# Lexmata/llama-gguf

Measured on AMD Instinct MI355X. Metric: decode tokens/sec Llama-3-8B Q4_K_M, 1 GPU; % of HBM roofline, higher is better.
Workload: dtype f32 (x as 4xint8 limbs on the matrix cores, exact int32 accumulation)

## Files before the change

### llama-gguf_amd/csrc/attention.hip

```cpp
#include <cstdlib>

#include "attn_split.h"
#include "tq_fwht.h"
#include "xq.h"
#include "prefill.h"
#include "timeline.h"

LGH_TL_DEFINE(attn)

namespace lgh {

template <int D, int G, int NW, bool PF = false, bool DIRECT = false, bool MULTI = false>
__global__ void __launch_bounds__(NW * 64) attn_partial_kernel(const float* __restrict__ q, const float* __restrict__ kc,
                                                           const float* __restrict__ vc, uint32_t max_seq, float scale,
                                                           const int* pos_ptr, int kv_len_fixed, uint32_t n_splits,
                                                           float* __restrict__ part_ml, float* __restrict__ part_acc,
                                                           const int* __restrict__ slot = nullptr, uint64_t slot_stride = 0) {
  constexpr int LPR = D / 4;
  constexpr int RPW = 64 / LPR;
  __shared__ float s_ml[NW * G * 2];
  __shared__ __attribute__((aligned(16))) float s_acc[NW * G * D];
  LGH_TL_BEGIN(attn, lgh::TL_ATTN, n_splits);

  const uint32_t kvh = blockIdx.x / n_splits, sp = blockIdx.x % n_splits;
  const uint32_t lane = threadIdx.x & 63, wave = threadIdx.x >> 6;
  const uint32_t sub = lane / LPR, li = lane % LPR;
  uint32_t kv_len = (uint32_t)kv_len_fixed;
  if (PF) {
    kv_len += blockIdx.y;
    q += (size_t)blockIdx.y * gridDim.x * G * D;
  } else if (MULTI) {
    const uint32_t sq = blockIdx.y;
    uint32_t pw, sl;
    sload_u32x2(pos_ptr + sq, slot + sq, pw, sl);
    kv_len = pw + 1;
    q += (size_t)sq * (gridDim.x / n_splits) * G * D;
    kc += (size_t)sl * slot_stride;
    vc += (size_t)sl * slot_stride;
    part_ml += (size_t)sq * gridDim.x * G * 2;
    part_acc += (size_t)sq * gridDim.x * G * D;
  } else if (pos_ptr) {
    kv_len = sload_u32(pos_ptr) + 1;
  }

  f32x4 qv[G];
#pragma unroll
  for (int g = 0; g < G; g++) qv[g] = *reinterpret_cast<const f32x4*>(q + ((size_t)kvh * G + g) * D + li * 4);

  float m[G], l[G];
  f32x4 acc[G];
#pragma unroll
  for (int g = 0; g < G; g++) { m[g] = kNegBig; l[g] = 0.0f; acc[g] = (f32x4)(0.0f); }

  const float* kbase = kc + (size_t)kvh * max_seq * D + li * 4;
  const float* vbase = vc + (size_t)kvh * max_seq * D + li * 4;
  const uint32_t stride = n_splits * NW * RPW;
  auto row_of = [&](uint32_t base) { const uint32_t p = base + sub; return p < kv_len ? p : kv_len - 1; };
  auto step = [&](uint32_t base, f32x4 k4, f32x4 v4) { attn_step4<G, LPR>(qv, k4, v4, scale, base + sub < kv_len, m, l, acc); };
  constexpr int kAhead = 4;
  for (uint32_t base = (sp * NW + wave) * RPW; base < kv_len; base += kAhead * stride) {
    f32x4 kk[kAhead], vv[kAhead];
#pragma unroll
    for (int j = 0; j < kAhead; j++) {
      const uint32_t r = row_of(base + j * stride);
      kk[j] = __builtin_nontemporal_load(reinterpret_cast<const f32x4*>(kbase + (size_t)r * D));
      vv[j] = __builtin_nontemporal_load(reinterpret_cast<const f32x4*>(vbase + (size_t)r * D));
    }
#pragma unroll
    for (int j = 0; j < kAhead; j++)
      if (base + j * stride < kv_len) step(base + j * stride, kk[j], vv[j]);
  }

  attn_merge_rows<G, LPR>(m, l, acc);
  attn_stash<G, 4, LPR>(s_ml, s_acc, wave, sub, li, m, l, acc);
  __syncthreads();
  const size_t pbase = ((size_t)kvh * n_splits + sp) * G;
  for (uint32_t e = threadIdx.x; e < (uint32_t)(G * D); e += NW * 64) {
    const uint32_t g = e / D, dim = e % D;
    float mn, lsum, a;
    attn_merge_waves<NW, G, D>(s_ml, s_acc, g, dim, mn, lsum, a);
    if (DIRECT) {
      const float o = a * (1.0f / lsum);
      part_acc[(pbase + g) * D + dim] = o;
      if (part_ml) xq_store_chunk(reinterpret_cast<uint8_t*>(part_ml), (uint32_t)((pbase + g) * D + dim) >> 4, o);
    } else if (PF) {
      const _Float16 o = (_Float16)(a * (1.0f / lsum));
      *reinterpret_cast<_Float16*>(reinterpret_cast<uint8_t*>(part_acc) + xh_offset(blockIdx.y, (uint32_t)(pbase + g) * D + dim)) = o;
    } else {
      attn_store_partial<D>(part_ml, part_acc, pbase + g, dim, mn, lsum, a);
    }
  }
  LGH_TL_END();
}

__device__ __forceinline__ f32x4 unpack_i8x4(uint32_t w, float scale) {
  f32x4 r;
  r.x = (float)(int)(int8_t)(w & 0xFFu) * scale;
  r.y = (float)(int)(int8_t)((w >> 8) & 0xFFu) * scale;
  r.z = (float)(int)(int8_t)((w >> 16) & 0xFFu) * scale;
  r.w = (float)(int)(int8_t)(w >> 24) * scale;
  return r;
}

__device__ __forceinline__ float i8_row_scale(float amax) { return amax > 1e-10f ? amax / 127.0f : 1.0f; }
__device__ __forceinline__ uint32_t i8_quantize(float v, float scale) {
  float r = roundf(v / scale);
  r = r < -128.0f ? -128.0f : (r > 127.0f ? 127.0f : r);
  return (uint32_t)(int)r & 0xFFu;
}

template <int LPR>
__device__ __forceinline__ uint32_t quantize_row_i8(f32x4 x, float& scale) {
  float amax = fmaxf(fmaxf(fabsf(x.x), fabsf(x.y)), fmaxf(fabsf(x.z), fabsf(x.w)));
  amax = fmaxf(amax, dpp_f<0xB1>(amax));
  amax = fmaxf(amax, dpp_f<0x4E>(amax));
  amax = fmaxf(amax, dpp_f<0x141>(amax));
  amax = fmaxf(amax, dpp_f<0x140>(amax));
  if (LPR == 32) amax = fmaxf(amax, __shfl_xor(amax, 16, 64));
  scale = i8_row_scale(amax);
  return i8_quantize(x.x, scale) | i8_quantize(x.y, scale) << 8 | i8_quantize(x.z, scale) << 16 | i8_quantize(x.w, scale) << 24;
}

template <int FMT>
__device__ __forceinline__ float fp8_decode(uint32_t b) {
  const uint32_t mag = b & 0x7Fu;
// ... 231 lines not shown
  hipStream_t st;
  uint32_t n_seq; const int* slot; uint64_t slot_stride;
};

template <int D, int G, int NW>
static hipError_t attn_go(const AttnArgs& a) {
  const dim3 grid(a.n_kv * a.n_splits, a.n_seq ? a.n_seq : 1);
  if (a.n_seq)
    hipLaunchKernelGGL((attn_partial_kernel<D, G, NW, false, false, true>), grid, dim3(NW * 64), 0, a.st, a.q, a.kc, a.vc, a.max_seq, a.scale, a.pos, 0,
                       a.n_splits, a.part_ml, a.part_acc, a.slot, a.slot_stride);
  else
    hipLaunchKernelGGL((attn_partial_kernel<D, G, NW>), grid, dim3(NW * 64), 0, a.st, a.q, a.kc, a.vc, a.max_seq, a.scale, a.pos, a.kv_len_fixed,
                       a.n_splits, a.part_ml, a.part_acc);
  return hipGetLastError();
}

static hipError_t attn_split_dispatch(uint32_t head_dim, uint32_t g, const AttnArgs& a) {
  const bool long_ctx = (a.pos ? a.max_seq : (uint32_t)a.kv_len_fixed) >= 2048;
  return attn_dispatch(head_dim, g, [&](auto d, auto gg) {
    constexpr int D = decltype(d)::value, G = decltype(gg)::value;
    return long_ctx ? attn_go<D, G, 8>(a) : attn_go<D, G, 4>(a);
  });
}

hipError_t attn_launch(const float* q, const float* kcache, const float* vcache, uint32_t n_heads, uint32_t n_kv,
                       uint32_t head_dim, uint32_t max_seq, float scale, const int* pos, int kv_len_fixed,
                       uint32_t n_splits, float* part_ml, float* part_acc, hipStream_t st) {
  if (n_kv == 0 || n_heads % n_kv) return hipErrorInvalidValue;
  return attn_split_dispatch(head_dim, n_heads / n_kv,
                             AttnArgs{q, kcache, vcache, n_kv, max_seq, scale, pos, kv_len_fixed, n_splits, part_ml, part_acc, st, 0, nullptr, 0});
}

hipError_t attn_direct_launch(const float* q, const float* kcache, const float* vcache, uint32_t n_heads, uint32_t n_kv, uint32_t head_dim,
                              uint32_t max_seq, float scale, const int* pos, float* out, uint8_t* xq_out, hipStream_t st) {
  if (n_kv == 0 || n_heads % n_kv || !pos) return hipErrorInvalidValue;
  return attn_dispatch(head_dim, n_heads / n_kv, [&](auto d, auto gg) {
    hipLaunchKernelGGL((attn_partial_kernel<decltype(d)::value, decltype(gg)::value, 16, false, true>), dim3(n_kv), dim3(1024), 0, st, q, kcache, vcache,
                       max_seq, scale, pos, 0, 1u, reinterpret_cast<float*>(xq_out), out);
    return hipGetLastError();
  });
}

struct PfTqEpi { const float* signs; float inv_scale, inv_d; };

template <int D, int NW, bool TQ>
__global__ void __launch_bounds__(NW * 64) attn_pf_mfma_kernel(const float* __restrict__ q, const float* __restrict__ kc, const float* __restrict__ vc,
                                                               uint32_t n_heads, uint32_t g_per_kv, uint32_t max_seq, float scale, uint32_t pos0,
                                                               uint32_t m_tokens, uint8_t* __restrict__ xh_out, const PfTqEpi tq) {
  constexpr int DJ = D / 4;
  constexpr int DQ = D / 16;
  constexpr int DP = D + 4;
  extern __shared__ __attribute__((aligned(16))) float pf_lds[];
  float (*s_o)[16][DP] = reinterpret_cast<float (*)[16][DP]>(pf_lds);
  float (*s_m)[16] = reinterpret_cast<float (*)[16]>(pf_lds + NW * 16 * DP);
  float (*s_l)[16] = s_m + NW;
  const uint32_t head = blockIdx.x, tt = blockIdx.y, kvh = head / g_per_kv;
  const uint32_t lane = threadIdx.x & 63, wave = threadIdx.x >> 6, n = lane & 15, c = lane >> 4;
  const uint32_t tok = tt * 16 + n, tokc = tok < m_tokens ? tok : m_tokens - 1;
  const uint32_t kv_last = pos0 + m_tokens - 1;
  const uint32_t n_tiles = (pos0 + tt * 16 + 16 + 15) / 16;
  float qf[DJ];
  {
    const float* qp = q + ((size_t)tokc * n_heads + head) * D + c * DJ;
#pragma unroll
    for (int j = 0; j < DJ; j += 4) {
      const f32x4 v = *reinterpret_cast<const f32x4*>(qp + j);
      qf[j] = v.x; qf[j + 1] = v.y; qf[j + 2] = v.z; qf[j + 3] = v.w;
    }
  }
  const float* kbase = kc + (size_t)kvh * max_seq * D;
  const float* vbase = vc + (size_t)kvh * max_seq * D;
// ... 243 lines not shown
```

### llama-gguf_amd/csrc/common.h

```cpp
#pragma once

#include <hip/hip_runtime.h>
#include <stdint.h>
#include <stddef.h>
#include <vector>

#include "../../include/llama_gguf_hip.h"

namespace lgh {

typedef uint32_t u32x4 __attribute__((ext_vector_type(4)));
typedef uint32_t u32x2 __attribute__((ext_vector_type(2)));
typedef float f32x4 __attribute__((ext_vector_type(4)));

constexpr int kWave = 64;
constexpr int kNumCU = 256;

__host__ __device__ inline uint32_t blk_elems(int t) {
  switch (t) {
    case LGH_TYPE_F32: case LGH_TYPE_F16: case LGH_TYPE_BF16: return 1;
    case LGH_TYPE_Q4_0: case LGH_TYPE_Q4_1: case LGH_TYPE_Q5_0: case LGH_TYPE_Q5_1: case LGH_TYPE_Q8_0:
    case LGH_TYPE_Q8_1: return 32;
    case LGH_TYPE_Q2_K: case LGH_TYPE_Q3_K: case LGH_TYPE_Q4_K: case LGH_TYPE_Q5_K: case LGH_TYPE_Q6_K:
    case LGH_TYPE_Q8_K: return 256;
// ... 148 lines not shown
hipError_t embed_launch(int src_type, const uint8_t* table, const int* token, float* dst, uint32_t hidden, int* state,
                        uint8_t* xq, const float* xq_nw, float* xq_ssq, hipStream_t st);

hipError_t rms_norm_launch(const float* x, const float* w, float eps, float* out, uint32_t n, hipStream_t st);
hipError_t rope_launch(float* q, float* k, uint32_t n_heads, uint32_t n_kv, uint32_t head_dim, const int* pos,
                       const float* rope_cs, int neox, hipStream_t st);
hipError_t embed_multi_launch(int src_type, const uint8_t* table, const int* tokens, float* dst, uint32_t hidden, uint32_t n_seq, uint8_t* xq,
                              const float* xq_nw, float* xq_ssq, uint32_t xq_stride, uint32_t ssq_stride, hipStream_t st);
hipError_t argmax_multi_launch(const float* logits, uint32_t n, uint32_t n_seq, float* part_val, int* part_idx, int* next, hipStream_t st);
hipError_t attn_multi_launch(const float* q, const float* kcache, const float* vcache, uint32_t n_heads, uint32_t n_kv, uint32_t head_dim,
                             uint32_t max_seq, float scale, const int* pos, const int* slot, uint64_t slot_stride, uint32_t n_seq,
                             uint32_t n_splits, float* part_ml, float* part_acc, hipStream_t st);
hipError_t attn_combine_multi_launch(const float* part_ml, const float* part_acc, uint32_t n_heads, uint32_t n_kv, uint32_t head_dim,
                                     uint32_t n_splits, uint32_t n_seq, float* out, uint8_t* xq_out, hipStream_t st);
hipError_t ewise_launch(int op, const float* a, const float* b, float s, float* out, uint64_t n, hipStream_t st);
hipError_t softmax_rows_launch(const float* x, float* out, uint32_t rows, uint32_t last_dim, hipStream_t st);
hipError_t matmul_f32_launch(const float* a, const float* b, float* c, uint32_t m, uint32_t k, uint32_t n, hipStream_t st);
hipError_t silu_mul_launch(const float* gate, const float* up, float* out, uint32_t n, hipStream_t st);
hipError_t argmax_launch(const float* logits, uint32_t n, float* part_val, int* part_idx, int* state, int* out_token,
                         hipStream_t st);
hipError_t argmax_merge_launch(const float* part_val, const int* part_idx, uint32_t nparts, int* state, int* out_token, hipStream_t st);
hipError_t advance_launch(int* state, hipStream_t st);
hipError_t copy_words_launch(void* dst, const void* src, uint32_t n_words, hipStream_t st);
hipError_t moe_group_launch(const int* sel, uint32_t n_seq, uint32_t top_k, uint32_t n_experts, int* cnt, int* idx, uint32_t idx_stride, hipStream_t st);
hipError_t moe_combine_launch(const float* tmp, const float* moe_w, uint32_t top_k, float* hidden, uint32_t H, uint32_t n_seq, const float* nw,
                              uint8_t* xq, uint32_t xq_stride, float* ssq, uint32_t ssq_stride, hipStream_t st);
hipError_t moe_router_launch(const float* x, const float* norm_w, float eps, const float* w, uint32_t hidden,
                             uint32_t n_experts, uint32_t top_k, int* sel, float* sel_w, hipStream_t st, uint32_t n_tokens = 1);

hipError_t attn_launch(const float* q, const float* kcache, const float* vcache, uint32_t n_heads, uint32_t n_kv,
                       uint32_t head_dim, uint32_t max_seq, float scale, const int* pos, int kv_len_fixed,
                       uint32_t n_splits, float* part_ml, float* part_acc, hipStream_t st);
hipError_t attn_direct_launch(const float* q, const float* kcache, const float* vcache, uint32_t n_heads, uint32_t n_kv, uint32_t head_dim,
                              uint32_t max_seq, float scale, const int* pos, float* out, uint8_t* xq_out, hipStream_t st);
bool attn_shape_has_fast_kernel(uint32_t head_dim, uint32_t group);
hipError_t kv_roundtrip_launch(int fmt, const float* x, uint32_t n, uint8_t* bytes, float* scale_out, float* back, hipStream_t st);
hipError_t attn_q8_launch(int fmt, const float* q, int8_t* k8, int8_t* v8, float* kscale, float* vscale, const float* k_new, const float* v_new,
                          uint32_t n_heads, uint32_t n_kv, uint32_t head_dim, uint32_t max_seq, float scale, const int* pos, uint32_t n_splits,
                          float* part_ml, float* part_acc, hipStream_t st);
hipError_t attn_q8_multi_launch(int fmt, const float* q, int8_t* k8, int8_t* v8, float* kscale, float* vscale, const float* k_new, const float* v_new,
                                uint32_t x_stride, uint32_t n_heads, uint32_t n_kv, uint32_t head_dim, uint32_t max_seq, float scale, const int* pos,
                                const int* slot, uint32_t n_seq, uint32_t n_splits, float* part_ml, float* part_acc, hipStream_t st);
hipError_t attn_tq_launch(int bits, const float* q, uint8_t* kq, uint8_t* vq, const float* k_new, const float* v_new, const float* signs,
                          uint32_t n_heads, uint32_t n_kv, uint32_t head_dim, uint32_t max_seq, float scale, const int* pos, uint32_t n_splits,
                          float* part_ml, float* part_acc, hipStream_t st, const float* qjl_s = nullptr, uint32_t* kx = nullptr);
hipError_t attn_tq_combine_launch(int bits, const float* part_ml, const float* part_acc, const float* signs, uint32_t n_heads, uint32_t n_kv,
                                  uint32_t head_dim, uint32_t n_splits, float* out, uint8_t* xq_out, hipStream_t st, uint32_t n_seq = 0,
                                  uint32_t xq_stride = 0);
hipError_t attn_tq_multi_launch(int bits, const float* q, uint8_t* kq, uint8_t* vq, const float* k_new, const float* v_new, const float* signs,
                                uint32_t n_heads, uint32_t n_kv, uint32_t head_dim, uint32_t max_seq, float scale, const int* pos, const int* slot,
                                uint64_t code_stride, uint64_t x_stride, uint32_t kv_stride, uint32_t n_seq, uint32_t n_splits, float* part_ml,
                                float* part_acc, hipStream_t st, const float* qjl_s = nullptr, uint32_t* kx = nullptr);
hipError_t tq_compress_launch(int bits, const float* x, uint32_t dim, const float* signs, uint8_t* out, hipStream_t st, const float* qjl_s = nullptr,
                              uint32_t* qjl_out = nullptr);
uint32_t tq_row_bytes_host(int bits, uint32_t d);
hipError_t tq_pf_rows_launch(int bits, float* kscr, float* vscr, uint8_t* kq, uint8_t* vq, float* q, const float* signs, uint32_t n_heads,
                             uint32_t n_kv, uint32_t head_dim, uint32_t max_seq, uint32_t pos0, uint32_t m_store, uint32_t m_q, uint32_t n_expand,
                             hipStream_t st);
hipError_t attn_prefill_tq_launch(const float* q, const float* kscr, const float* vscr, const float* signs, uint32_t n_heads, uint32_t n_kv,
                                  uint32_t head_dim, uint32_t max_seq, float scale, uint32_t pos0, uint32_t m_tokens, uint8_t* xh_out, hipStream_t st);
hipError_t attn_decode_any_launch(const float* q, const float* kcache, const float* vcache, float* out, uint32_t n_heads, uint32_t n_kv,
                                  uint32_t head_dim, uint32_t max_seq, float scale, const int* pos, hipStream_t st);
hipError_t attn_generic_launch(const float* q, const float* k, const float* v, float* out, uint32_t n_heads, uint32_t n_kv, uint32_t seq_len,
                               uint32_t kv_len, uint32_t kv_rows, uint32_t d, float scale, hipStream_t st);
hipError_t attn_combine_launch(const float* part_ml, const float* part_acc, uint32_t n_heads, uint32_t n_kv,
                               uint32_t head_dim, uint32_t n_splits, float* out, uint8_t* xq_out, hipStream_t st);

// ... 15 lines not shown
```

### llama-gguf_amd/csrc/engine.h

```cpp
#pragma once

#include <functional>
#include <string>
#include <vector>

#include "common.h"
#include "kv_cache.h"
#include "sample.h"

namespace lgh {

struct LayerW {
  bool owned = false;
  DevWeight wq, wk, wv, wo, gate, up, down;
  DevWeight gate_exps, up_exps, down_exps;
  float* attn_norm = nullptr;
  float* ffn_norm = nullptr;
  float* router = nullptr;
  float* bq = nullptr; float* bk = nullptr; float* bv = nullptr; float* bo = nullptr;
  KvCache kv;
  bool moe() const { return router != nullptr; }
};

enum TokenMode { MODE_PREFILL = 0, MODE_FORWARD = 1, MODE_GREEDY = 2, MODE_SAMPLE = 3, MODE_COUNT = 4 };
// ... 35 lines not shown
  SampBufs samp;
  std::vector<lgh_sampler_config_ex> samp_cfg;
  std::vector<uint8_t> samp_set;
};

}

struct lgh_ctx {
  lgh_model_desc d{};
  lgh::KvLayout kvl;
  int device = 0;
  uint32_t l0 = 0, l1 = 0;
  bool first = true, last = true;
  hipStream_t own_stream = nullptr, stream = nullptr;
  std::vector<lgh::LayerW> layers;
  uint8_t* embd_raw = nullptr;
  int embd_type = -1;
  size_t embd_bytes = 0;
  std::vector<uint8_t> embd_host;
  lgh::DevWeight output;
  float* output_norm = nullptr;
  void *fwd_hidden = nullptr, *fwd_token = nullptr;
  float *hidden = nullptr, *xnorm = nullptr, *q = nullptr, *kv_tmp = nullptr, *attn_out = nullptr, *act = nullptr,
        *act2 = nullptr, *logits = nullptr, *part_ml = nullptr, *part_acc = nullptr, *rope_cs = nullptr, *moe_w = nullptr,
        *amax_v = nullptr;
  int *moe_sel = nullptr, *state = nullptr, *amax_i = nullptr, *tok_log = nullptr;
  uint32_t n_splits = 8;
  size_t pos = 0;
  bool finalized = false;
  bool profiling = false;
  std::string err;
  hipGraphExec_t graph[lgh::MODE_COUNT][2] = {};
  bool attn_direct = false;
  bool attn_generic = false;
  uint32_t direct_attn_max_kv = 0;
  uint64_t graph_nodes = 0;
  lgh_stats stats{};
  std::vector<lgh::ProfRec> prof;
  std::vector<void*> allocs;
  std::vector<lgh::XqBuf> xqs;
  lgh::PfScratch pf;
  lgh::BatchScratch batch;
  float* tq_signs = nullptr;
  std::vector<float> tq_signs_host;
  float* tq_qjl = nullptr;
  std::vector<float> tq_qjl_host;
  float* kv_shift_tmp = nullptr;
  lgh::SampBufs samp;
  lgh_sampler_config_ex samp_cfg{};
  bool samp_set = false;
};

#include <cstring>

int fail(lgh_ctx* c, int status, const std::string& msg);
#define HIP_TRY(c, status, expr)                                                                      \
  do {                                                                                                \
    hipError_t e__ = (expr);                                                                          \
    if (e__ != hipSuccess)                                                                            \
      return fail((c), (status), std::string(#expr) + ": " + hipGetErrorString(e__));                 \
  } while (0)

struct LayoutInfo {
  int dev_type;
  int nplanes;
  uint32_t bpb[4];
// ... 128 lines not shown
```

### llama-gguf_amd/csrc/engine.hip

```cpp
#include "engine.h"
#include "prefill.h"
#include "xq.h"

#include <algorithm>
#include <cmath>
#include <cstdlib>
#include <cstring>

using namespace lgh;

constexpr uint32_t kDirectAttnDefaultKv = 64;

static int warm_kernels(lgh_ctx* c) {
  if (c->d.flags & LGH_FLAG_NO_GRAPH) return LGH_OK;
  int rc = LGH_OK;
  const bool keep_direct = c->attn_direct;
  for (int v = 0; v < 2 && !rc; v++) {
    if (v == 1 && c->direct_attn_max_kv == 0) continue;
    c->attn_direct = v == 1;
    HIP_TRY(c, LGH_OPERATION_FAILED, hipMemsetAsync(c->state, 0, ST_WORDS * 4, c->stream));
    for (int mode : {c->last ? MODE_GREEDY : MODE_PREFILL, MODE_PREFILL})
      if (!rc) rc = enqueue_token(c, mode);
  }
  c->attn_direct = keep_direct;
  for (auto& q : c->xqs) q.fresh = false;
  if (rc) return rc;
  if (c->samp.ctl && (rc = samp_warm(c, c->samp, c->logits, 1))) return rc;
  HIP_TRY(c, LGH_OPERATION_FAILED, hipMemsetAsync(c->state, 0, ST_WORDS * 4, c->stream));
  HIP_TRY(c, LGH_OPERATION_FAILED, hipStreamSynchronize(c->stream));
  return LGH_OK;
}

static int ensure_graph(lgh_ctx* c, int mode) {
  const int var = c->attn_direct ? 1 : 0;
  if (c->graph[mode][var]) return LGH_OK;
  size_t n_nodes = 0;
  const int rc = capture_graph(c, &c->graph[mode][var], [&] { return enqueue_token(c, mode); }, &n_nodes);
  if (n_nodes && (mode == MODE_GREEDY || (c->graph_nodes == 0 && mode != MODE_SAMPLE))) c->graph_nodes = n_nodes;
  return rc;
}

static int step(lgh_ctx* c, int mode) {
  if (c->pos >= c->d.max_seq_len)
    return fail(c, LGH_INVALID_ARGUMENT, "position " + std::to_string(c->pos) + " >= max_seq_len " + std::to_string(c->d.max_seq_len));
// ... 750 lines not shown
```

### llama-gguf_amd/csrc/engine_layer.hip

```cpp
#include "engine.h"
#include "xq.h"

#include <algorithm>
#include <cmath>

using namespace lgh;

namespace lgh {
hipError_t kv_store_launch(const float* k, const float* v, float* kcache, float* vcache, uint32_t n_kv, uint32_t d,
                           uint32_t max_seq, const int* pos, hipStream_t st);
}

void rope_table_host(const lgh_model_desc& d, std::vector<float>& cs) {
  const uint32_t half = d.head_dim / 2;
  cs.assign((size_t)d.max_seq_len * half * 2, 0.0f);
  for (uint32_t p = 0; p < d.max_seq_len; p++) {
    const float position = (float)p / d.rope_freq_scale;
    for (uint32_t i = 0; i < half; i++) {
      const float freq = 1.0f / std::pow(d.rope_freq_base, (float)(2 * i) / (float)d.head_dim);
      const float theta = position * freq;
      cs[((size_t)p * half + i) * 2] = std::cos(theta);
      cs[((size_t)p * half + i) * 2 + 1] = std::sin(theta);
    }
  }
// ... 123 lines not shown
  auto merge = [&](uint8_t* img) {
    return run_k(c, LGH_K_ATTN_COMBINE, LGH_SYM_ATTN_COMBINE, 0, [&] {
      return attn_combine_launch(c->part_ml, c->part_acc, d.num_heads, d.num_kv_heads, d.head_dim, c->n_splits, v.attn_out, img, c->stream);
    });
  };
  if (kvl.tq()) {
    const int bits = kvl.tq_bits();
    const float* signs = c->tq_signs + (size_t)(li - c->l0) * d.num_kv_heads * 2 * d.head_dim;
    const bool qjl = kvl.qjl();
    const float* qjl_s = qjl ? c->tq_qjl + (size_t)(li - c->l0) * d.num_kv_heads * d.head_dim * d.head_dim : nullptr;
    if ((rc = run_k(c, LGH_K_ATTN, LGH_SYM_ATTN, kv_bytes, [&] {
           return attn_tq_launch(bits, v.q, kv.k_bytes(), kv.v_bytes(), k_new, v_new, signs, d.num_heads, d.num_kv_heads, d.head_dim, d.max_seq_len,
                                 scale, pos, c->n_splits, c->part_ml, c->part_acc, c->stream, qjl_s, qjl ? kv.kx() : nullptr);
         })))
      return rc;
    uint8_t* const img = image();
    rc = run_k(c, LGH_K_ATTN_COMBINE, LGH_SYM_ATTN_COMBINE, 0, [&] {
      return attn_tq_combine_launch(bits, c->part_ml, c->part_acc, signs, d.num_heads, d.num_kv_heads, d.head_dim, c->n_splits, v.attn_out, img, c->stream);
    });
  } else if (kvl.staged()) {
    if ((rc = run_k(c, LGH_K_ATTN, LGH_SYM_ATTN, kv_bytes, [&] {
           return attn_q8_launch((int)d.kv_cache_type, v.q, kv.k_i8(), kv.v_i8(), kv.kscale(), kv.vscale(), k_new, v_new, d.num_heads, d.num_kv_heads, d.head_dim,
                                 d.max_seq_len, scale, pos, c->n_splits, c->part_ml, c->part_acc, c->stream);
         })))
      return rc;
    rc = merge(image());
  } else if (c->attn_generic) {
    rc = run_k(c, LGH_K_ATTN, LGH_SYM_ATTN, kv_bytes, [&] {
      return attn_decode_any_launch(v.q, kv.k_f32(), kv.v_f32(), v.attn_out, d.num_heads, d.num_kv_heads, d.head_dim, d.max_seq_len, scale, pos, c->stream);
    });
  } else if (c->attn_direct) {
    uint8_t* const img = image();
    rc = run_k(c, LGH_K_ATTN, LGH_SYM_ATTN, kv_bytes, [&] {
      return attn_direct_launch(v.q, kv.k_f32(), kv.v_f32(), d.num_heads, d.num_kv_heads, d.head_dim, d.max_seq_len, scale, pos, v.attn_out, img, c->stream);
    });
  } else {
    if ((rc = run_k(c, LGH_K_ATTN, LGH_SYM_ATTN, kv_bytes, [&] {
           return attn_launch(v.q, kv.k_f32(), kv.v_f32(), d.num_heads, d.num_kv_heads, d.head_dim, d.max_seq_len, scale, pos, 0, c->n_splits, c->part_ml,
                              c->part_acc, c->stream);
         })))
      return rc;
    rc = merge(image());
  }
  if (rc) return rc;
  if (qa) { qa->fresh = true; qa->tag = nullptr; }
  else xq_stale(c, v.attn_out);
  return LGH_OK;
}

static int layer_forward(lgh_ctx* c, uint32_t li, const float* next_nw, bool next_mfma) {
  LayerW& Lw = c->layers[li];
  const AttnView av{c->hidden, c->q, c->kv_tmp, c->attn_out};
  int rc;
  if ((rc = qkv_forward(c, Lw, av))) return rc;
  if ((rc = attention_forward(c, Lw, li, av, 1.0f / std::sqrt((float)c->d.head_dim), mfma_type(Lw.wo.type)))) return rc;
  const bool ffn_mfma = Lw.moe() ? mfma_type(Lw.gate_exps.type) : mfma_type(Lw.gate.type);
  if ((rc = linear_any(c, LGH_K_WO, Lw.wo, c->attn_out, c->hidden, nullptr, c->hidden, Lw.bo, ffn_mfma ? 2 : 0, Lw.ffn_norm))) return rc;
  if (c->profiling) {
    if ((rc = run_k(c, -1, -1, 0, [&] { return hipSuccess; }))) return rc;
  }
  return ffn_forward(c, Lw, FfnView{c->hidden, c->act, c->act2, c->xnorm, c->moe_sel, c->moe_w}, next_nw, next_mfma);
}

int embed_forward(lgh_ctx* c) {
  const lgh_model_desc& d = c->d;
  XqBuf* qh = nullptr;
  const float* nw0 = nullptr;
// ... 62 lines not shown
```

### llama-gguf_amd/csrc/ops_api.hip

```cpp
#include "engine.h"
#include "xq.h"
#include "prefill.h"

#include <cmath>
#include <vector>

using namespace lgh;

#include <algorithm>

#ifdef LGH_STAMPS
namespace lgh { hipError_t pf_read_stamps(unsigned long long* host, size_t n); }
extern "C" int lgh_debug_pf_stamps(unsigned long long* out, size_t n) { return lgh::pf_read_stamps(out, n) == hipSuccess ? 0 : 10; }
namespace lgh { hipError_t mv_read_stamps(unsigned long long* host, size_t n); hipError_t mvq_read_stamps(unsigned long long* host, size_t n); hipError_t mvq_read_wave_stamps(unsigned long long* host, size_t n); hipError_t mvq_spans(unsigned long long* host, int reset); }
#include <cstdio>
#include "timeline.h"
namespace lgh { hipError_t tl_read_mvq(void*); hipError_t tl_read_attn(void*); hipError_t tl_read_deq(void*); hipError_t tl_read_misc(void*); }
extern "C" long long lgh_debug_timeline(int which, void* out) {
  if (!out) return (long long)sizeof(lgh::TlBuf);
  hipError_t e = which == 0 ? lgh::tl_read_mvq(out) : which == 1 ? lgh::tl_read_attn(out) : which == 2 ? lgh::tl_read_deq(out) : lgh::tl_read_misc(out);
  return e == hipSuccess ? 0 : -1;
}
#endif

// ... 462 lines not shown
    if (host[kind] && l.pos_bytes(kind))
      if (int rc = down_bytes(t, host[kind], kv.t[kind], n_slots * l.slot_bytes(kind))) return rc;
  return LGH_OK;
}

int attn_image_down(Tmp& t, const float* attn_out, size_t qd, uint8_t* image_out) {
  const XqBuf* qa = xq_find(t.c, attn_out);
  if (!qa || !qa->fresh) return LGH_OPERATION_FAILED;
  return down_bytes(t, image_out, qa->xq, xq_bytes(qd));
}

int attn_multi_images(Tmp& t, size_t n_seq, size_t qd) {
  const size_t n = n_seq + 1, xb = n * xq_stride_of((uint32_t)qd), sf = n * ssq_stride_of((uint32_t)qd);
  uint8_t* xq = (uint8_t*)up_bytes(t, nullptr, xb);
  float* ssq = t.up(nullptr, sf);
  if (!xq || !ssq) return LGH_ALLOCATION_FAILED;
  if (hipMemsetD32Async((hipDeviceptr_t)xq, (int)0x7FC0BEEFu, xb / 4, t.c->stream) != hipSuccess ||
      hipMemsetD32Async((hipDeviceptr_t)ssq, (int)0x7FC0BEEFu, sf, t.c->stream) != hipSuccess)
    return LGH_OPERATION_FAILED;
  return register_views(t.c, t.c->batch.attn_out, xq, ssq, (uint32_t)qd, (uint32_t)n);
}

int attn_multi_images_down(Tmp& t, size_t n_seq, size_t qd, uint8_t* image_out) {
  const XqBuf* qa = xq_find(t.c, t.c->batch.attn_out);
  if (!qa || !qa->fresh) return LGH_OPERATION_FAILED;
  return down_bytes(t, image_out, qa->xq, (n_seq + 1) * xq_stride_of((uint32_t)qd));
}

int attn_run(Tmp& t, const AttnView& v, const void* const* up, void* const* down, float scale, float* out, uint8_t* image_out) {
  const size_t qd = (size_t)t.c->d.num_heads * t.c->d.head_dim;
  LayerW Lw;
  int rc;
  if ((rc = kv_upload(t, t.c->kvl, 1, up, Lw.kv))) return rc;
  if (attention_forward(t.c, Lw, 0, v, scale, image_out != nullptr)) return LGH_OPERATION_FAILED;
  if (image_out && (rc = attn_image_down(t, v.attn_out, qd, image_out))) return rc;
  if (down && (rc = kv_download(t, t.c->kvl, 1, down, Lw.kv))) return rc;
  return t.down(out, v.attn_out, qd);
}

int attn_multi_run(Tmp& t, size_t n_slots, size_t n_seq, const void* const* up, void* const* down, float scale, float* out, uint8_t* image_out) {
  BatchScratch& Bs = t.c->batch;
  const size_t qd = (size_t)t.c->d.num_heads * t.c->d.head_dim;
  int rc;
  if ((rc = kv_upload(t, t.c->kvl, n_slots, up, Bs.kv[0]))) return rc;
  if (image_out && (rc = attn_multi_images(t, n_seq, qd))) return rc;
  if (attention_forward_multi(t.c, 0, (uint32_t)n_seq, scale, image_out != nullptr)) return LGH_OPERATION_FAILED;
  if (image_out && (rc = attn_multi_images_down(t, n_seq, qd, image_out))) return rc;
  if (down && (rc = kv_download(t, t.c->kvl, n_slots, down, Bs.kv[0]))) return rc;
  return t.down(out, Bs.attn_out, n_seq * qd);
}

float half_to_float(uint16_t h) {
  const uint32_t s = (uint32_t)(h >> 15) << 31, e = (h >> 10) & 0x1Fu, m = h & 0x3FFu;
  float v;
  if (e == 0) v = (float)m * 0x1p-24f;
  else if (e == 31) v = m ? NAN : INFINITY;
  else v = std::ldexp((float)(m | 0x400u), (int)e - 25);
  uint32_t b;
  std::memcpy(&b, &v, 4);
  b |= s;
  std::memcpy(&v, &b, 4);
  return v;
}

}

extern "C" {

int lgh_op_attention_decode(int device, int path, const float* q, const float* k_cache, const float* v_cache, float* out, size_t n_heads,
                            size_t n_kv, size_t head_dim, size_t max_seq, float scale, size_t pos, int n_splits, uint8_t* image_out) {
  Tmp t(device);
  if (t.rc) return t.rc;
  if (!q || !k_cache || !v_cache || !out || n_kv == 0 || n_heads % n_kv || head_dim == 0 || pos >= max_seq || max_seq > 0x7FFFFFFFu)
    return LGH_INVALID_ARGUMENT;
  if (path < 0 || path > 2 || (path == 2 && image_out)) return LGH_INVALID_ARGUMENT;
  const size_t g = n_heads / n_kv;
  const bool fast = attn_shape_has_fast_kernel((uint32_t)head_dim, (uint32_t)g);
  if (path != 2 && !fast) return LGH_UNSUPPORTED;
  if (path == 0 && (n_splits < 1 || n_splits > 32)) return LGH_INVALID_ARGUMENT;
  if (path == 2 && max_seq * 4 > 150 * 1024) return LGH_UNSUPPORTED;
  const AttnView v{nullptr, t.up(q, n_heads * head_dim), nullptr, t.up(nullptr, n_heads * head_dim)};
  if (!v.q || !v.attn_out) return LGH_ALLOCATION_FAILED;
  int rc;
  if ((rc = attn_setup(t, LGH_KV_F32, n_heads, n_kv, head_dim, max_seq, path == 0 ? n_splits : 0)) || (rc = set_pos(t, pos))) return rc;
  t.c->attn_direct = path == 1;
  t.c->attn_generic = path == 2;
  const void* const caches[KV_KINDS] = {k_cache, v_cache};
  return attn_run(t, v, caches, nullptr, scale, out, image_out);
}

int lgh_op_attention_decode_multi(int device, const float* q, const float* k_cache, const float* v_cache, float* out, size_t n_heads, size_t n_kv,
                                  size_t head_dim, size_t max_seq, size_t n_slots, size_t n_seq, const int* pos, const int* slot, float scale,
                                  int n_splits, uint8_t* image_out) {
  Tmp t(device);
  if (t.rc) return t.rc;
  if (!q || !k_cache || !v_cache || !out || !pos || !slot || n_kv == 0 || n_heads % n_kv || head_dim == 0 || max_seq == 0 || max_seq > 0x7FFFFFFFu ||
      n_slots == 0 || n_splits < 1 || n_splits > 32 || !seqs_ok(n_seq, kMaxBatch, slot, n_slots, false, pos, max_seq))
    return LGH_INVALID_ARGUMENT;
  if (!attn_shape_has_fast_kernel((uint32_t)head_dim, (uint32_t)(n_heads / n_kv))) return LGH_UNSUPPORTED;
  if (int rc = attn_multi_setup(t, LGH_KV_F32, q, nullptr, nullptr, n_heads, n_kv, head_dim, max_seq, n_seq, pos, slot, n_splits)) return rc;
  const void* const caches[KV_KINDS] = {k_cache, v_cache};
  return attn_multi_run(t, n_slots, n_seq, caches, nullptr, scale, out, image_out);
}

int lgh_op_attention_kv8(int device, uint32_t kv_cache_type, const float* q, int8_t* k_bytes, int8_t* v_bytes, float* k_scale, float* v_scale,
                         const float* k_new, const float* v_new, float* out, size_t n_heads, size_t n_kv, size_t head_dim, size_t max_seq,
                         float scale, size_t pos, int n_splits, uint8_t* image_out) {
  Tmp t(device);
  if (t.rc) return t.rc;
  if (kv_cache_type < LGH_KV_INT8 || kv_cache_type > LGH_KV_FP8_E5M2) return LGH_UNSUPPORTED;
  const bool i8 = kv_cache_type == LGH_KV_INT8;
  if (!q || !k_bytes || !v_bytes || !k_new || !v_new || !out || (i8 && (!k_scale || !v_scale))) return LGH_INVALID_ARGUMENT;
  if (n_kv == 0 || n_heads % n_kv || pos >= max_seq || max_seq > 0x7FFFFFFFu || n_splits < 1 || n_splits > 32) return LGH_INVALID_ARGUMENT;
  if (!attn_shape_has_fast_kernel((uint32_t)head_dim, (uint32_t)(n_heads / n_kv))) return LGH_UNSUPPORTED;
  const AttnView v{nullptr, t.up(q, n_heads * head_dim), up_kv_new(t, k_new, v_new, n_kv * head_dim), t.up(nullptr, n_heads * head_dim)};
  if (!v.q || !v.kv_tmp || !v.attn_out) return LGH_ALLOCATION_FAILED;
  int rc;
  if ((rc = attn_setup(t, kv_cache_type, n_heads, n_kv, head_dim, max_seq, n_splits)) || (rc = set_pos(t, pos))) return rc;
// ... 1177 lines not shown
```

### llama-gguf_amd/hip_backend.py

```python
from __future__ import annotations

import ctypes as C
import os
from typing import Iterable, Optional, Sequence

import numpy as np

_HERE = os.path.dirname(os.path.abspath(__file__))
LIB_PATH = os.path.join(_HERE, "lib", "libllama_gguf_hip%s.so" % ("_" + os.environ["LGH_LIB_VARIANT"] if os.environ.get("LGH_LIB_VARIANT") else ""))

ABI_SYMBOLS = (
    "lgh_device_count", "lgh_create", "lgh_upload_tensor", "lgh_finalize", "lgh_destroy", "lgh_forward",
    "lgh_prefill_token", "lgh_prefill_batch", "lgh_prefill_is_batched", "lgh_op_mat_mat",
    "lgh_op_kv_roundtrip", "lgh_op_add", "lgh_op_mul", "lgh_op_scale", "lgh_op_silu", "lgh_op_gelu", "lgh_op_softmax", "lgh_op_matmul", "lgh_op_matvec",
    "lgh_op_matvec_q", "lgh_op_attention", "lgh_backend_create", "lgh_backend_destroy", "lgh_backend_load_weight",
    "lgh_backend_has_weight", "lgh_backend_vec_mat_q", "lgh_backend_last_error", "lgh_reset", "lgh_position", "lgh_kv_truncate", "lgh_kv_shift_left", "lgh_stage_prefill_batch", "lgh_stage_hidden_block_buffer", "lgh_forward_argmax", "lgh_decode_greedy",
    "lgh_last_error", "lgh_get_stats", "lgh_set_profiling", "lgh_set_stream", "lgh_get_stream", "lgh_synchronize",
    "lgh_read_hidden", "lgh_stage_hidden_buffer", "lgh_stage_forward", "lgh_op_dequantize", "lgh_op_vec_mat",
    "lgh_op_rms_norm", "lgh_op_rope", "lgh_op_attention_cached", "lgh_op_silu_mul", "lgh_op_norm_vec_mat",
    "lgh_op_swiglu_vec_mat", "lgh_bench_vec_mat", "lgh_bench_hbm_read", "lgh_gguf_inspect", "lgh_load_gguf",
    "lgh_stage_io_buffers", "lgh_stage_set_forward_targets", "lgh_stage_step", "lgh_stage_read_tokens", "lgh_gguf_get", "lgh_stage_read_logits",
    "lgh_pipeline_create", "lgh_pipeline_upload_tensor", "lgh_pipeline_finalize", "lgh_pipeline_destroy", "lgh_pipeline_forward",
    "lgh_pipeline_prefill_token", "lgh_pipeline_decode_greedy", "lgh_pipeline_reset", "lgh_pipeline_position", "lgh_pipeline_kv_truncate", "lgh_pipeline_stages",
    "lgh_pipeline_last_error",
# ... 736 lines not shown
                      device: int = 0) -> np.ndarray:
    wg, wu, x = np.ascontiguousarray(w_gate), np.ascontiguousarray(w_up), _f32(x)
    nw = _f32(norm_w) if norm_w is not None else None
    out = np.empty(n, dtype=np.float32)
    _chk(load_library().lgh_op_swiglu_vec_mat(device, ggml_type, wg.ctypes.data, wu.ctypes.data, x.ctypes.data,
                                              nw.ctypes.data if nw is not None else None, eps, out.ctypes.data,
                                              x.size, n), "swiglu_vec_mat")
    return out


def op_rms_norm(x, w, eps: float, device: int = 0) -> np.ndarray:
    x, w = _f32(x), _f32(w)
    out = np.empty_like(x)
    _chk(load_library().lgh_op_rms_norm(device, x.ctypes.data, w.ctypes.data, eps, out.ctypes.data, x.size), "rms_norm")
    return out


def op_rope(q, k, pos: int, freq_base: float, freq_scale: float, neox: bool, device: int = 0):
    q, k = _f32(q).copy(), _f32(k).copy()
    _chk(load_library().lgh_op_rope(device, q.ctypes.data, k.ctypes.data, q.shape[0], k.shape[0], q.shape[1], pos,
                                    freq_base, freq_scale, int(neox)), "rope")
    return q, k


def op_attention_cached(q, k_cache, v_cache, scale: float, kv_len: int, n_splits: int = 8, device: int = 0) -> np.ndarray:
    q, kc, vc = _f32(q), _f32(k_cache), _f32(v_cache)
    out = np.empty_like(q)
    _chk(load_library().lgh_op_attention_cached(device, q.ctypes.data, kc.ctypes.data, vc.ctypes.data, out.ctypes.data,
                                                q.shape[0], kc.shape[0], q.shape[1], kc.shape[1], scale, kv_len,
                                                n_splits), "attention_cached")
    return out


ATTN_SPLIT, ATTN_DIRECT, ATTN_ANY = 0, 1, 2


def _attn_image(q, n_images: int = 1):
    nb = _xq_bytes(q.shape[-2] * q.shape[-1])
    return np.zeros(nb if n_images == 1 else (n_images, nb), np.uint8)


def op_attention_decode(path: int, q, k_cache, v_cache, scale: float, pos: int, n_splits: int = 8, device: int = 0, *, image: bool = False):
    q, kc, vc = _f32(q), _f32(k_cache), _f32(v_cache)
    out = np.empty_like(q)
    img = _attn_image(q) if image else None
    _chk(load_library().lgh_op_attention_decode(device, path, q.ctypes.data, kc.ctypes.data, vc.ctypes.data, out.ctypes.data, q.shape[0],
                                                kc.shape[0], q.shape[1], kc.shape[1], scale, pos, n_splits, _ptr(img)), "attention_decode")
    return (out, img) if image else out


def op_attention_decode_multi(q, k_cache, v_cache, scale: float, pos, slot, n_splits: int = 8, device: int = 0, *, image: bool = False):
    q, kc, vc = _f32(q), _f32(k_cache), _f32(v_cache)
    pos, slot = np.ascontiguousarray(pos, dtype=np.int32), np.ascontiguousarray(slot, dtype=np.int32)
    out = np.empty_like(q)
    img = _attn_image(q, q.shape[0] + 1) if image else None
    _chk(load_library().lgh_op_attention_decode_multi(device, q.ctypes.data, kc.ctypes.data, vc.ctypes.data, out.ctypes.data, q.shape[1],
                                                      kc.shape[1], q.shape[2], kc.shape[2], kc.shape[0], q.shape[0], pos.ctypes.data,
                                                      slot.ctypes.data, scale, n_splits, _ptr(img)), "attention_decode_multi")
    return (out, img) if image else out


def _ptr(a):
    return None if a is None else a.ctypes.data


def op_qkv_rope(types, ws, biases, x, norm_w, eps: float, head_dim: int, n_heads: int, n_kv: int, k_cache, v_cache, pos: int,
                rope_base: float, rope_scale: float, device: int = 0):
# ... 668 lines not shown
```

Before: 689.6.

## Launch direct decode attention per query head and raise its kv-length cutoff

The single-launch direct attention path now runs one 1024-thread workgroup per query head (GW=1) instead of one per kv head, so the grid has n_heads workgroups rather than n_kv and keeps more compute units busy during short-context decode. Each workgroup reloads the shared K/V rows of its group, which multiplies KV cache reads by the group size. The threshold for using the direct path is raised from 64 to 192 positions. The old per-kv-head launch stays available as a separate path for testing.

```diff
diff --git a/llama-gguf_amd/csrc/attention.hip b/llama-gguf_amd/csrc/attention.hip
--- a/llama-gguf_amd/csrc/attention.hip
+++ b/llama-gguf_amd/csrc/attention.hip
@@ -10,19 +10,20 @@
 
 namespace lgh {
 
-template <int D, int G, int NW, bool PF = false, bool DIRECT = false, bool MULTI = false>
-__global__ void __launch_bounds__(NW * 64) attn_partial_kernel(const float* __restrict__ q, const float* __restrict__ kc,
-                                                           const float* __restrict__ vc, uint32_t max_seq, float scale,
-                                                           const int* pos_ptr, int kv_len_fixed, uint32_t n_splits,
-                                                           float* __restrict__ part_ml, float* __restrict__ part_acc,
-                                                           const int* __restrict__ slot = nullptr, uint64_t slot_stride = 0) {
+template <int D, int G, int NW, bool PF, bool DIRECT, bool MULTI, int GW>
+__device__ __forceinline__ void attn_partial_body(const float* __restrict__ q, const float* __restrict__ kc, const float* __restrict__ vc,
+                                                  uint32_t max_seq, float scale, const int* pos_ptr, int kv_len_fixed, uint32_t n_splits,
+                                                  float* __restrict__ part_ml, float* __restrict__ part_acc, const int* __restrict__ slot,
+                                                  uint64_t slot_stride) {
+  static_assert(GW == G || (DIRECT && GW >= 1 && G % GW == 0), "only the single-launch form splits a kv group over workgroups");
   constexpr int LPR = D / 4;
   constexpr int RPW = 64 / LPR;
-  __shared__ float s_ml[NW * G * 2];
-  __shared__ __attribute__((aligned(16))) float s_acc[NW * G * D];
+  __shared__ float s_ml[NW * GW * 2];
+  __shared__ __attribute__((aligned(16))) float s_acc[NW * GW * D];
   LGH_TL_BEGIN(attn, lgh::TL_ATTN, n_splits);
 
-  const uint32_t kvh = blockIdx.x / n_splits, sp = blockIdx.x % n_splits;
+  const uint32_t hg = blockIdx.x / n_splits, sp = blockIdx.x % n_splits;
+  const uint32_t kvh = GW == G ? hg : hg * GW / G;
   const uint32_t lane = threadIdx.x & 63, wave = threadIdx.x >> 6;
   const uint32_t sub = lane / LPR, li = lane % LPR;
   uint32_t kv_len = (uint32_t)kv_len_fixed;
@@ -43,20 +44,20 @@
     kv_len = sload_u32(pos_ptr) + 1;
   }
 
-  f32x4 qv[G];
-#pragma unroll
-  for (int g = 0; g < G; g++) qv[g] = *reinterpret_cast<const f32x4*>(q + ((size_t)kvh * G + g) * D + li * 4);
-
-  float m[G], l[G];
-  f32x4 acc[G];
-#pragma unroll
-  for (int g = 0; g < G; g++) { m[g] = kNegBig; l[g] = 0.0f; acc[g] = (f32x4)(0.0f); }
+  f32x4 qv[GW];
+#pragma unroll
+  for (int g = 0; g < GW; g++) qv[g] = *reinterpret_cast<const f32x4*>(q + ((size_t)hg * GW + g) * D + li * 4);
+
+  float m[GW], l[GW];
+  f32x4 acc[GW];
+#pragma unroll
+  for (int g = 0; g < GW; g++) { m[g] = kNegBig; l[g] = 0.0f; acc[g] = (f32x4)(0.0f); }
 
   const float* kbase = kc + (size_t)kvh * max_seq * D + li * 4;
   const float* vbase = vc + (size_t)kvh * max_seq * D + li * 4;
   const uint32_t stride = n_splits * NW * RPW;
   auto row_of = [&](uint32_t base) { const uint32_t p = base + sub; return p < kv_len ? p : kv_len - 1; };
-  auto step = [&](uint32_t base, f32x4 k4, f32x4 v4) { attn_step4<G, LPR>(qv, k4, v4, scale, base + sub < kv_len, m, l, acc); };
+  auto step = [&](uint32_t base, f32x4 k4, f32x4 v4) { attn_step4<GW, LPR>(qv, k4, v4, scale, base + sub < kv_len, m, l, acc); };
   constexpr int kAhead = 4;
   for (uint32_t base = (sp * NW + wave) * RPW; base < kv_len; base += kAhead * stride) {
     f32x4 kk[kAhead], vv[kAhead];
@@ -71,14 +72,14 @@
       if (base + j * stride < kv_len) step(base + j * stride, kk[j], vv[j]);
   }
 
-  attn_merge_rows<G, LPR>(m, l, acc);
-  attn_stash<G, 4, LPR>(s_ml, s_acc, wave, sub, li, m, l, acc);
+  attn_merge_rows<GW, LPR>(m, l, acc);
+  attn_stash<GW, 4, LPR>(s_ml, s_acc, wave, sub, li, m, l, acc);
   __syncthreads();
-  const size_t pbase = ((size_t)kvh * n_splits + sp) * G;
-  for (uint32_t e = threadIdx.x; e < (uint32_t)(G * D); e += NW * 64) {
+  const size_t pbase = ((size_t)hg * n_splits + sp) * GW;
+  for (uint32_t e = threadIdx.x; e < (uint32_t)(GW * D); e += NW * 64) {
     const uint32_t g = e / D, dim = e % D;
     float mn, lsum, a;
-    attn_merge_waves<NW, G, D>(s_ml, s_acc, g, dim, mn, lsum, a);
+    attn_merge_waves<NW, GW, D>(s_ml, s_acc, g, dim, mn, lsum, a);
     if (DIRECT) {
       const float o = a * (1.0f / lsum);
       part_acc[(pbase + g) * D + dim] = o;
@@ -91,6 +92,22 @@
     }
   }
   LGH_TL_END();
+}
+
+template <int D, int G, int NW, bool PF = false, bool DIRECT = false, bool MULTI = false>
+__global__ void __launch_bounds__(NW * 64) attn_partial_kernel(const float* __restrict__ q, const float* __restrict__ kc,
+                                                           const float* __restrict__ vc, uint32_t max_seq, float scale,
+                                                           const int* pos_ptr, int kv_len_fixed, uint32_t n_splits,
+                                                           float* __restrict__ part_ml, float* __restrict__ part_acc,
+                                                           const int* __restrict__ slot = nullptr, uint64_t slot_stride = 0) {
+  attn_partial_body<D, G, NW, PF, DIRECT, MULTI, G>(q, kc, vc, max_seq, scale, pos_ptr, kv_len_fixed, n_splits, part_ml, part_acc, slot, slot_stride);
+}
+
+template <int D, int G, int GW>
+__global__ void __launch_bounds__(1024) attn_direct_head_kernel(const float* __restrict__ q, const float* __restrict__ kc, const float* __restrict__ vc,
+                                                                uint32_t max_seq, float scale, const int* pos_ptr, float* __restrict__ xq_out,
+                                                                float* __restrict__ out) {
+  attn_partial_body<D, G, 16, false, true, false, GW>(q, kc, vc, max_seq, scale, pos_ptr, 0, 1u, xq_out, out, nullptr, 0);
 }
 
 __device__ __forceinline__ f32x4 unpack_i8x4(uint32_t w, float scale) {
@@ -388,11 +405,16 @@
 }
 
 hipError_t attn_direct_launch(const float* q, const float* kcache, const float* vcache, uint32_t n_heads, uint32_t n_kv, uint32_t head_dim,
-                              uint32_t max_seq, float scale, const int* pos, float* out, uint8_t* xq_out, hipStream_t st) {
+                              uint32_t max_seq, float scale, const int* pos, float* out, uint8_t* xq_out, hipStream_t st, bool per_kv_head) {
   if (n_kv == 0 || n_heads % n_kv || !pos) return hipErrorInvalidValue;
   return attn_dispatch(head_dim, n_heads / n_kv, [&](auto d, auto gg) {
-    hipLaunchKernelGGL((attn_partial_kernel<decltype(d)::value, decltype(gg)::value, 16, false, true>), dim3(n_kv), dim3(1024), 0, st, q, kcache, vcache,
-                       max_seq, scale, pos, 0, 1u, reinterpret_cast<float*>(xq_out), out);
+    constexpr int D = decltype(d)::value, G = decltype(gg)::value;
+    if (per_kv_head)
+      hipLaunchKernelGGL((attn_partial_kernel<D, G, 16, false, true>), dim3(n_kv), dim3(1024), 0, st, q, kcache, vcache, max_seq, scale, pos, 0, 1u,
+                         reinterpret_cast<float*>(xq_out), out);
+    else
+      hipLaunchKernelGGL((attn_direct_head_kernel<D, G, 1>), dim3(n_heads), dim3(1024), 0, st, q, kcache, vcache, max_seq, scale, pos,
+                         reinterpret_cast<float*>(xq_out), out);
     return hipGetLastError();
   });
 }
diff --git a/llama-gguf_amd/csrc/common.h b/llama-gguf_amd/csrc/common.h
--- a/llama-gguf_amd/csrc/common.h
+++ b/llama-gguf_amd/csrc/common.h
@@ -204,7 +204,7 @@
                        uint32_t head_dim, uint32_t max_seq, float scale, const int* pos, int kv_len_fixed,
                        uint32_t n_splits, float* part_ml, float* part_acc, hipStream_t st);
 hipError_t attn_direct_launch(const float* q, const float* kcache, const float* vcache, uint32_t n_heads, uint32_t n_kv, uint32_t head_dim,
-                              uint32_t max_seq, float scale, const int* pos, float* out, uint8_t* xq_out, hipStream_t st);
+                              uint32_t max_seq, float scale, const int* pos, float* out, uint8_t* xq_out, hipStream_t st, bool per_kv_head = false);
 bool attn_shape_has_fast_kernel(uint32_t head_dim, uint32_t group);
 hipError_t kv_roundtrip_launch(int fmt, const float* x, uint32_t n, uint8_t* bytes, float* scale_out, float* back, hipStream_t st);
 hipError_t attn_q8_launch(int fmt, const float* q, int8_t* k8, int8_t* v8, float* kscale, float* vscale, const float* k_new, const float* v_new,
diff --git a/llama-gguf_amd/csrc/engine.h b/llama-gguf_amd/csrc/engine.h
--- a/llama-gguf_amd/csrc/engine.h
+++ b/llama-gguf_amd/csrc/engine.h
@@ -91,6 +91,7 @@
   std::string err;
   hipGraphExec_t graph[lgh::MODE_COUNT][2] = {};
   bool attn_direct = false;
+  bool attn_direct_per_kv = false;
   bool attn_generic = false;
   uint32_t direct_attn_max_kv = 0;
   uint64_t graph_nodes = 0;
diff --git a/llama-gguf_amd/csrc/engine.hip b/llama-gguf_amd/csrc/engine.hip
--- a/llama-gguf_amd/csrc/engine.hip
+++ b/llama-gguf_amd/csrc/engine.hip
@@ -9,7 +9,7 @@
 
 using namespace lgh;
 
-constexpr uint32_t kDirectAttnDefaultKv = 64;
+constexpr uint32_t kDirectAttnDefaultKv = 192;
 
 static int warm_kernels(lgh_ctx* c) {
   if (c->d.flags & LGH_FLAG_NO_GRAPH) return LGH_OK;
diff --git a/llama-gguf_amd/csrc/engine_layer.hip b/llama-gguf_amd/csrc/engine_layer.hip
--- a/llama-gguf_amd/csrc/engine_layer.hip
+++ b/llama-gguf_amd/csrc/engine_layer.hip
@@ -179,7 +179,8 @@
   } else if (c->attn_direct) {
     uint8_t* const img = image();
     rc = run_k(c, LGH_K_ATTN, LGH_SYM_ATTN, kv_bytes, [&] {
-      return attn_direct_launch(v.q, kv.k_f32(), kv.v_f32(), d.num_heads, d.num_kv_heads, d.head_dim, d.max_seq_len, scale, pos, v.attn_out, img, c->stream);
+      return attn_direct_launch(v.q, kv.k_f32(), kv.v_f32(), d.num_heads, d.num_kv_heads, d.head_dim, d.max_seq_len, scale, pos, v.attn_out, img, c->stream,
+                                c->attn_direct_per_kv);
     });
   } else {
     if ((rc = run_k(c, LGH_K_ATTN, LGH_SYM_ATTN, kv_bytes, [&] {
diff --git a/llama-gguf_amd/csrc/ops_api.hip b/llama-gguf_amd/csrc/ops_api.hip
--- a/llama-gguf_amd/csrc/ops_api.hip
+++ b/llama-gguf_amd/csrc/ops_api.hip
@@ -518,6 +518,11 @@
   LayerW Lw;
   int rc;
   if ((rc = kv_upload(t, t.c->kvl, 1, up, Lw.kv))) return rc;
+  if (image_out) {
+    const XqBuf* qa = xq_get(t.c, v.attn_out, (uint32_t)qd);
+    if (!qa) return LGH_ALLOCATION_FAILED;
+    if (hipMemsetD32Async((hipDeviceptr_t)qa->xq, (int)0x7FC0BEEFu, xq_bytes(qd) / 4, t.c->stream) != hipSuccess) return LGH_OPERATION_FAILED;
+  }
   if (attention_forward(t.c, Lw, 0, v, scale, image_out != nullptr)) return LGH_OPERATION_FAILED;
   if (image_out && (rc = attn_image_down(t, v.attn_out, qd, image_out))) return rc;
   if (down && (rc = kv_download(t, t.c->kvl, 1, down, Lw.kv))) return rc;
@@ -559,7 +564,7 @@
   if (t.rc) return t.rc;
   if (!q || !k_cache || !v_cache || !out || n_kv == 0 || n_heads % n_kv || head_dim == 0 || pos >= max_seq || max_seq > 0x7FFFFFFFu)
     return LGH_INVALID_ARGUMENT;
-  if (path < 0 || path > 2 || (path == 2 && image_out)) return LGH_INVALID_ARGUMENT;
+  if (path < 0 || path > 3 || (path == 2 && image_out)) return LGH_INVALID_ARGUMENT;
   const size_t g = n_heads / n_kv;
   const bool fast = attn_shape_has_fast_kernel((uint32_t)head_dim, (uint32_t)g);
   if (path != 2 && !fast) return LGH_UNSUPPORTED;
@@ -569,7 +574,8 @@
   if (!v.q || !v.attn_out) return LGH_ALLOCATION_FAILED;
   int rc;
   if ((rc = attn_setup(t, LGH_KV_F32, n_heads, n_kv, head_dim, max_seq, path == 0 ? n_splits : 0)) || (rc = set_pos(t, pos))) return rc;
-  t.c->attn_direct = path == 1;
+  t.c->attn_direct = path == 1 || path == 3;
+  t.c->attn_direct_per_kv = path == 3;
   t.c->attn_generic = path == 2;
   const void* const caches[KV_KINDS] = {k_cache, v_cache};
   return attn_run(t, v, caches, nullptr, scale, out, image_out);
diff --git a/llama-gguf_amd/hip_backend.py b/llama-gguf_amd/hip_backend.py
--- a/llama-gguf_amd/hip_backend.py
+++ b/llama-gguf_amd/hip_backend.py
@@ -792,7 +792,7 @@
     return out
 
 
-ATTN_SPLIT, ATTN_DIRECT, ATTN_ANY = 0, 1, 2
+ATTN_SPLIT, ATTN_DIRECT, ATTN_ANY, ATTN_DIRECT_PER_KV = 0, 1, 2, 3
 
 
 def _attn_image(q, n_images: int = 1):
```

Result: no change. 689.9, median of 2 (+0.0%).
